# wanmeihuali/taichi_3d_gaussian_splatting

Hardware: NVIDIA H100
Metric: rendered Mpix/sec fwd+bwd @1080p, 1e6 Gaussians (higher is better)
Workload: dtype f32

## Files before the change

taichi_3d_gaussian_splatting_b200/csrc/api.cu:

```cuda
#include <cstdarg>
#include <cstdio>
#include <cstring>

#include "common.cuh"

namespace gsb {

static thread_local char g_error[512] = "";

void set_error(const char *fmt, ...) {
    va_list ap;
    va_start(ap, fmt);
    vsnprintf(g_error, sizeof(g_error), fmt, ap);
    va_end(ap);
}

static inline int64_t align_up(int64_t v, int64_t a) { return (v + a - 1) / a * a; }

static int bit_width(uint64_t v) {
    int b = 0;
    while (v) {
        ++b;
        v >>= 1;
    }
// ... 151 lines not shown
}

using namespace gsb;

extern "C" {

int gsb200_version(void) { return GSB200_VERSION; }

const char *gsb200_last_error(void) { return g_error; }

void gsb200_abi_sizes(int64_t *out3) {
    out3[0] = (int64_t)sizeof(GsbWorkspaceLayout);
    out3[1] = (int64_t)sizeof(GsbForwardArgs);
    out3[2] = (int64_t)sizeof(GsbBackwardArgs);
}

void gsb200_abi_sizes_ext(int64_t *out, int32_t n) {
    const int64_t all[5] = {(int64_t)sizeof(GsbWorkspaceLayout), (int64_t)sizeof(GsbForwardArgs), (int64_t)sizeof(GsbBackwardArgs),
                            (int64_t)sizeof(GsbExpandArgs), (int64_t)sizeof(GsbTrainStepArgs)};
    for (int i = 0; i < n && i < 5; ++i) out[i] = all[i];
}

int gsb200_workspace_layout(int64_t num_points, int32_t num_objects, int64_t key_capacity,
                            int32_t camera_height, int32_t camera_width, float far_plane,
                            float depth_to_sort_key_scale, uint32_t flags, GsbWorkspaceLayout *out) {
    return compute_layout(num_points, num_objects, key_capacity, camera_height, camera_width, far_plane,
                          depth_to_sort_key_scale, flags, out);
}

int gsb200_stage_preprocess(const GsbForwardArgs *a) {
    Workspace ws;
    int rc = resolve_fwd(a, &ws);
    if (rc != GSB_OK) return rc;
    cudaStream_t st = static_cast<cudaStream_t>(a->stream);
    GSB_CUDA_CHECK(cudaMemsetAsync(a->workspace, 0, (size_t)ws.layout.zero_bytes, st));
    return launch_preprocess(*a, ws, st);
}

int gsb200_stage_sort(const GsbForwardArgs *a) {
    Workspace ws;
    int rc = resolve_fwd(a, &ws);
    if (rc != GSB_OK) return rc;
    return launch_sort(ws, a->key_capacity, static_cast<cudaStream_t>(a->stream));
}

int gsb200_stage_tile_ranges(const GsbForwardArgs *a) {
    Workspace ws;
    int rc = resolve_fwd(a, &ws);
    if (rc != GSB_OK) return rc;
    const int T = (a->camera_height / GSB_TILE_HEIGHT) * (a->camera_width / GSB_TILE_WIDTH);
    return launch_tile_ranges(ws, a->key_capacity, T, static_cast<cudaStream_t>(a->stream));
}

int gsb200_stage_blend(const GsbForwardArgs *a) {
    Workspace ws;
    int rc = resolve_fwd(a, &ws);
    if (rc != GSB_OK) return rc;
    return launch_blend_forward(*a, ws, static_cast<cudaStream_t>(a->stream));
}

int gsb200_forward(const GsbForwardArgs *a) {
    Workspace ws;
    int rc = resolve_fwd(a, &ws);
    if (rc != GSB_OK) return rc;
    cudaStream_t st = static_cast<cudaStream_t>(a->stream);
    GSB_CUDA_CHECK(cudaMemsetAsync(a->workspace, 0, (size_t)ws.layout.zero_bytes, st));
    if ((rc = launch_preprocess(*a, ws, st)) != GSB_OK) return rc;
    if (a->host_counters && a->host_counters_event) {
        GSB_CUDA_CHECK(cudaMemcpyAsync(a->host_counters, ws.counters, 4 * sizeof(int64_t), cudaMemcpyDeviceToHost, st));
        GSB_CUDA_CHECK(cudaEventRecord(static_cast<cudaEvent_t>(a->host_counters_event), st));
    }
    if ((rc = launch_sort(ws, a->key_capacity, st)) != GSB_OK) return rc;
    const int T = (a->camera_height / GSB_TILE_HEIGHT) * (a->camera_width / GSB_TILE_WIDTH);
    if ((rc = launch_tile_ranges(ws, a->key_capacity, T, st)) != GSB_OK) return rc;
    return launch_blend_forward(*a, ws, st);
}

static int backward_impl(const GsbBackwardArgs *a, bool skip_on_overflow) {
    if (!a) {
        set_error("backward: args is null");
        return GSB_EINVAL;
    }
    const bool compact = (a->flags & GSB_FLAG_COMPACT_GRADS) != 0;
    if (!a->grad_rasterized_image || !a->pixel_accumulated_alpha ||
        !a->pixel_offset_of_last_effective_point || !a->magnitude_grad_viewspace_on_image ||
        !a->camera_intrinsics ||
        (a->num_points > 0 && (!a->pointcloud || !a->pointcloud_features || !a->point_object_id || !a->t_pointcloud_camera)) ||
        (a->num_points > 0 && !compact && (!a->grad_pointcloud || !a->grad_pointcloud_features)) ||
        (a->num_points > 0 && compact && (!a->grad_sum_compact || !a->grad_color_compact))) {
        set_error("backward: null pointer argument");
        return GSB_EINVAL;
    }
    {
        const void *ctl[6] = {a->ctl_accumulated_num_in_camera, a->ctl_accumulated_num_pixels,
                              a->ctl_accumulated_view_space_position_gradients,
                              a->ctl_accumulated_view_space_position_gradients_avg, a->ctl_accumulated_position_gradients,
                              a->ctl_accumulated_position_gradients_norm};
        int set = 0;
        for (const void *c : ctl) set += c != nullptr;
// ... 87 lines not shown
    cudaStream_t st;
    bool ok = true;
    explicit StageTimer(cudaStream_t s) : st(s) {
        for (auto &e : ev) ok = ok && cudaEventCreate(&e) == cudaSuccess;
    }
    ~StageTimer() {
        for (auto &e : ev) cudaEventDestroy(e);
    }
    void mark() {
        if (n < 9) cudaEventRecord(ev[n++], st);
    }
    int finish(float *out) {
        if (cudaStreamSynchronize(st) != cudaSuccess) return GSB_ECUDA;
        for (int i = 0; i < 8; ++i) out[i] = 0.0f;
        for (int i = 0; i + 1 < n; ++i) cudaEventElapsedTime(&out[i], ev[i], ev[i + 1]);
        return GSB_OK;
    }
};
}

int gsb200_forward_timed(const GsbForwardArgs *a, float *stage_ms_out) {
    Workspace ws;
    int rc = resolve_fwd(a, &ws);
    if (rc != GSB_OK) return rc;
    if (!stage_ms_out) return GSB_EINVAL;
    cudaStream_t st = static_cast<cudaStream_t>(a->stream);
    StageTimer t(st);
    if (!t.ok) {
        set_error("forward_timed: cudaEventCreate failed");
        return GSB_ECUDA;
    }
    const int T = (a->camera_height / GSB_TILE_HEIGHT) * (a->camera_width / GSB_TILE_WIDTH);
    t.mark();
    GSB_CUDA_CHECK(cudaMemsetAsync(a->workspace, 0, (size_t)ws.layout.zero_bytes, st));
    t.mark();
    if ((rc = launch_preprocess(*a, ws, st)) != GSB_OK) return rc;
    t.mark();
    if ((rc = launch_sort(ws, a->key_capacity, st)) != GSB_OK) return rc;
    t.mark();
    if ((rc = launch_tile_ranges(ws, a->key_capacity, T, st)) != GSB_OK) return rc;
    t.mark();
    if ((rc = launch_blend_forward(*a, ws, st)) != GSB_OK) return rc;
    t.mark();
    return t.finish(stage_ms_out);
}

int gsb200_backward_timed(const GsbBackwardArgs *a, float *stage_ms_out) {
    if (!a || !stage_ms_out) return GSB_EINVAL;
    Workspace ws;
    int rc = resolve_workspace(a->workspace, a->workspace_bytes, a->num_points, a->num_objects,
                               a->key_capacity, a->camera_height, a->camera_width, a->far_plane,
                               a->depth_to_sort_key_scale, a->flags, &ws);
    if (rc != GSB_OK) return rc;
    cudaStream_t st = static_cast<cudaStream_t>(a->stream);
    StageTimer t(st);
    if (!t.ok) {
        set_error("backward_timed: cudaEventCreate failed");
        return GSB_ECUDA;
    }
    t.mark();
    if (a->accum_rows > 0)
        GSB_CUDA_CHECK(cudaMemsetAsync(a->accum, 0, (size_t)a->accum_rows * GSB_ACCUM_FLOATS * 4, st));
    t.mark();
    if ((rc = launch_blend_backward(*a, ws, st)) != GSB_OK) return rc;
    t.mark();
    if ((rc = launch_backward_points(*a, ws, st)) != GSB_OK) return rc;
    t.mark();
// ... 99 lines not shown
}

int gsb200_sort_pairs(const void *keys_in, const int32_t *vals_in, void *keys_out, int32_t *vals_out,
                      int64_t n, int32_t key_bytes, int32_t end_bit, void *temp, int64_t temp_bytes,
                      void *stream) {
    if (n < 0 || (key_bytes != 4 && key_bytes != 8) || end_bit < 1 || end_bit > key_bytes * 8) {
        set_error("sort_pairs: bad arguments (n=%lld key_bytes=%d end_bit=%d)", (long long)n, key_bytes, end_bit);
        return GSB_EINVAL;
    }
    if (n == 0) return GSB_OK;
    if (n >= (1LL << 30)) {
        set_error("sort_pairs: n must be < 2^30");
        return GSB_EUNSUPPORTED;
    }
    if (!keys_in || !vals_in || !keys_out || !vals_out || !temp || temp_bytes < gsb200_sort_temp_bytes(n, key_bytes)) {
        set_error("sort_pairs: null pointer or temp too small");
        return GSB_EINVAL;
    }
    if (reinterpret_cast<uintptr_t>(keys_in) % 16 != 0 || reinterpret_cast<uintptr_t>(temp) % 256 != 0) {
        set_error("sort_pairs: keys_in must be 16-byte aligned and temp 256-byte aligned");
        return GSB_EINVAL;
    }
    cudaStream_t st = static_cast<cudaStream_t>(stream);
    const int64_t padded = align_up(n, SORT_TILE);
    const int64_t blocks = padded / SORT_TILE;
    char *b = static_cast<char *>(temp);
    long long *n_dev = reinterpret_cast<long long *>(b);
    unsigned int *tickets = reinterpret_cast<unsigned int *>(b + 256);
    unsigned int *hist = reinterpret_cast<unsigned int *>(b + 512);
    unsigned int *state = reinterpret_cast<unsigned int *>(b + 512 + 8 * 1024 * 4);
    const int64_t state_bytes = align_up(8 * blocks * 1024 * 4, 256);
    void *tmp_keys = b + 512 + 8 * 1024 * 4 + state_bytes;
    int *tmp_vals = reinterpret_cast<int *>(static_cast<char *>(tmp_keys) + align_up(padded * key_bytes, 256));
    GSB_CUDA_CHECK(cudaMemsetAsync(b, 0, (size_t)(512 + 8 * 1024 * 4 + state_bytes), st));
    const long long n_host = n;
    GSB_CUDA_CHECK(cudaMemcpyAsync(n_dev, &n_host, sizeof(n_host), cudaMemcpyHostToDevice, st));
    return sort_pairs_device(keys_in, vals_in, keys_out, vals_out, n_dev, padded, key_bytes, 0, end_bit, nullptr, hist,
                             state, tickets, tmp_keys, tmp_vals, st);
}

int gsb200_render_host(const GsbForwardArgs *device_args, const float *host_q, const float *host_t,
                       const float *host_K, float *staging, float *host_image_out,
                       int64_t *host_counters_out) {
    if (!device_args || !host_q || !host_t || !host_K || !staging || !host_image_out) {
        set_error("render_host: null pointer argument");
        return GSB_EINVAL;
    }
    GsbForwardArgs a = *device_args;
    cudaStream_t st = static_cast<cudaStream_t>(a.stream);
    const int n = a.num_objects;
    float *d_q = staging, *d_t = staging + 4 * n, *d_K = staging + 7 * n;
    GSB_CUDA_CHECK(cudaMemcpyAsync(d_q, host_q, sizeof(float) * 4 * n, cudaMemcpyHostToDevice, st));
    GSB_CUDA_CHECK(cudaMemcpyAsync(d_t, host_t, sizeof(float) * 3 * n, cudaMemcpyHostToDevice, st));
    GSB_CUDA_CHECK(cudaMemcpyAsync(d_K, host_K, sizeof(float) * 9, cudaMemcpyHostToDevice, st));
    a.q_pointcloud_camera = d_q;
    a.t_pointcloud_camera = d_t;
    a.camera_intrinsics = d_K;
    int rc = gsb200_forward(&a);
    if (rc != GSB_OK) return rc;
    GSB_CUDA_CHECK(cudaMemcpyAsync(host_image_out, a.rasterized_image,
                                   sizeof(float) * 3 * (size_t)a.camera_height * a.camera_width,
                                   cudaMemcpyDeviceToHost, st));
    if (host_counters_out)
        GSB_CUDA_CHECK(cudaMemcpyAsync(host_counters_out, a.workspace, sizeof(int64_t) * 4,
                                       cudaMemcpyDeviceToHost, st));
    GSB_CUDA_CHECK(cudaStreamSynchronize(st));
    return GSB_OK;
// ... 4 lines not shown
```

taichi_3d_gaussian_splatting_b200/csrc/common.cuh:

```cuda
#pragma once
#include <cuda_runtime.h>
#include <stdint.h>

#include "../../include/gsb200.h"

#define GSB_TILE_PIXELS (GSB_TILE_WIDTH * GSB_TILE_HEIGHT)

namespace gsb {

void set_error(const char *fmt, ...);
#define GSB_CUDA_CHECK(expr)                                                                   \
    do {                                                                                       \
        cudaError_t _e = (expr);                                                               \
        if (_e != cudaSuccess) {                                                               \
            gsb::set_error("%s failed: %s (%s:%d)", #expr, cudaGetErrorString(_e), __FILE__,   \
                           __LINE__);                                                          \
            return GSB_ECUDA;                                                                  \
        }                                                                                      \
    } while (0)

enum Counter { CNT_M = 0, CNT_K = 1, CNT_OVERFLOW = 2, CNT_MAX_DEPTH_KEY = 4 };
enum Ticket { TICKET_SCAN = 0, TICKET_SORT0 = 1  };

struct PoseBlock {
// ... 146 lines not shown
    return m;
}
#endif

#if defined(__CUDACC__) || defined(GSB_HOST_EMU)
constexpr float GSB_L2E = 1.4426950408889634f;
#ifdef GSB_HOST_EMU
__device__ __forceinline__ float ex2_mufu(float x) { return exp2f(x); }
#else
__device__ __forceinline__ float ex2_mufu(float x) {
    float y;
    asm("ex2.approx.ftz.f32 %0, %1;" : "=f"(y) : "f"(x));
    return y;
}
#endif
__device__ __forceinline__ float fast_alpha(float dx, float dy, float A, float B, float C, float ro) {
    return ex2_mufu(fmaf(dx, fmaf(A, dx, B * dy), (C * dy) * dy)) * ro;
}
__device__ __forceinline__ void fast_planes(const float4 r0, const float4 r1, float4 &s0, float4 &s1) {
    s0 = make_float4(r0.x, r0.y, (-0.5f * GSB_L2E) * r0.z, -GSB_L2E * r0.w);
    s1 = make_float4((-0.5f * GSB_L2E) * r1.x, r1.y * r1.z, 1.0f - r1.z, r1.w);
}
#endif

#if defined(__CUDACC__) || defined(GSB_HOST_EMU)
#ifdef GSB_HOST_EMU
__device__ __forceinline__ void mbar_init(unsigned long long *bar, unsigned int) { *bar = 0; }
__device__ __forceinline__ void mbar_arrive_expect_tx(unsigned long long *, unsigned int) {}
__device__ __forceinline__ void bulk_copy_g2s(void *dst_smem, const void *src_gmem, unsigned int bytes,
                                              unsigned long long *) {
    memcpy(dst_smem, src_gmem, bytes);
}
__device__ __forceinline__ void mbar_wait(unsigned long long *, unsigned int) { simt_emu::warp_exchange(0u); }
#else
__device__ __forceinline__ unsigned int smem_addr(const void *p) {
    return (unsigned int)__cvta_generic_to_shared(p);
}
__device__ __forceinline__ void mbar_init(unsigned long long *bar, unsigned int count) {
    asm volatile("mbarrier.init.shared::cta.b64 [%0], %1;" ::"r"(smem_addr(bar)), "r"(count));
    asm volatile("fence.mbarrier_init.release.cluster;" ::: "memory");
}
__device__ __forceinline__ void mbar_arrive_expect_tx(unsigned long long *bar, unsigned int bytes) {
    asm volatile("mbarrier.arrive.expect_tx.shared::cta.b64 _, [%0], %1;" ::"r"(smem_addr(bar)),
                 "r"(bytes)
                 : "memory");
}
__device__ __forceinline__ void bulk_copy_g2s(void *dst_smem, const void *src_gmem, unsigned int bytes,
                                              unsigned long long *bar) {
    asm volatile(
        "cp.async.bulk.shared::cluster.global.mbarrier::complete_tx::bytes [%0], [%1], %2, [%3];" ::"r"(
            smem_addr(dst_smem)),
        "l"(src_gmem), "r"(bytes), "r"(smem_addr(bar))
        : "memory");
}
__device__ __forceinline__ void mbar_wait(unsigned long long *bar, unsigned int parity) {
    asm volatile(
        "{\n"
        ".reg .pred p;\n"
        "WAIT_LOOP:\n"
        "mbarrier.try_wait.parity.shared::cta.b64 p, [%0], %1;\n"
        "@p bra WAIT_DONE;\n"
        "bra WAIT_LOOP;\n"
        "WAIT_DONE:\n"
        "}\n" ::"r"(smem_addr(bar)),
        "r"(parity)
        : "memory");
}
#endif

#endif

#ifdef GSB_HOST_EMU
#define GSB_EMU_COUNT(slot, n) (simt_emu::counters()[slot] += (long long)(n))
#else
#define GSB_EMU_COUNT(slot, n) ((void)0)
#endif
enum EmuCounter {
    EC_BF_VISITS = 0,
    EC_BF_VISITS_ANY = 1,
    EC_BF_PAIRS = 2,
    EC_TB_SPLATS = 3,
    EC_TB_CHUNKS = 4,
    EC_TB_ROWS = 5,
    EC_BATCHES = 6,
    EC_FW_VISITS = 7,
    EC_FW_PAIRS = 8,
};

static inline int num_sms() {
    static int n = 0;
    if (n == 0) {
        int dev = 0;
        cudaGetDevice(&dev);
        cudaDeviceGetAttribute(&n, cudaDevAttrMultiProcessorCount, dev);
        if (n <= 0) n = 132;
    }
    return n;
}

}
// ... 1 lines not shown
```

taichi_3d_gaussian_splatting_b200/csrc/preprocess.cu:

```cuda
#include "common.cuh"

namespace gsb {

template <int AR, int AC, int BC>
__device__ __forceinline__ void matmul(const float *a, const float *b, float *out) {
#pragma unroll
    for (int i = 0; i < AR; ++i)
#pragma unroll
        for (int j = 0; j < BC; ++j) {
            float s = a[i * AC] * b[j];
#pragma unroll
            for (int k = 1; k < AC; ++k) s = s + a[i * AC + k] * b[k * BC + j];
            out[i * BC + j] = s;
        }
}

__device__ __forceinline__ void rotation_from_quaternion(float x, float y, float z, float w, float *R) {
    float xx = x * x, yy = y * y, zz = z * z;
    float xy = x * y, xz = x * z, yz = y * z;
    float wx = w * x, wy = w * y, wz = w * z;
    R[0] = 1 - 2 * (yy + zz); R[1] = 2 * (xy - wz);     R[2] = 2 * (xz + wy);
    R[3] = 2 * (xy + wz);     R[4] = 1 - 2 * (xx + zz); R[5] = 2 * (yz - wx);
    R[6] = 2 * (xz - wy);     R[7] = 2 * (yz + wx);     R[8] = 1 - 2 * (xx + yy);
}

__device__ __forceinline__ float exp_cr(float x) { return (float)exp((double)x); }
__device__ __forceinline__ float sigmoid_cr(float x) { return 1.0f / (1.0f + exp_cr(-x)); }

__device__ __forceinline__ void quat_mul(const float *a, const float *b, float *o) {
    float x0 = a[0], y0 = a[1], z0 = a[2], w0 = a[3];
    float x1 = b[0], y1 = b[1], z1 = b[2], w1 = b[3];
    o[0] = w0 * x1 + x0 * w1 + y0 * z1 - z0 * y1;
    o[1] = w0 * y1 - x0 * z1 + y0 * w1 + z0 * x1;
    o[2] = w0 * z1 + x0 * y1 - y0 * x1 + z0 * w1;
    o[3] = w0 * w1 - x0 * x1 - y0 * y1 - z0 * z1;
}

__global__ void pose_kernel(const float *__restrict__ q_pc, const float *__restrict__ t_pc, int n_obj,
                            PoseBlock *__restrict__ poses) {
    int o = blockIdx.x * blockDim.x + threadIdx.x;
    if (o >= n_obj) return;
    float qi[4] = {-q_pc[4 * o], -q_pc[4 * o + 1], -q_pc[4 * o + 2], q_pc[4 * o + 3]};
    float t[3] = {t_pc[3 * o], t_pc[3 * o + 1], t_pc[3 * o + 2]};
    float n = sqrtf(((qi[0] * qi[0] + qi[1] * qi[1]) + qi[2] * qi[2]) + qi[3] * qi[3]);
    float qn[4] = {qi[0] / n, qi[1] / n, qi[2] / n, qi[3] / n};
    float v[4] = {t[0], t[1], t[2], 0.0f};
    float qc[4] = {-qn[0], -qn[1], -qn[2], qn[3]};
    float tmp[4], rot[4];
    quat_mul(qn, v, tmp);
    quat_mul(tmp, qc, rot);
    float ti[3] = {-rot[0], -rot[1], -rot[2]};
    float R[9];
    rotation_from_quaternion(qi[0], qi[1], qi[2], qi[3], R);
    PoseBlock pb;
    pb.T[0] = R[0]; pb.T[1] = R[1]; pb.T[2] = R[2];  pb.T[3] = ti[0];
    pb.T[4] = R[3]; pb.T[5] = R[4]; pb.T[6] = R[5];  pb.T[7] = ti[1];
    pb.T[8] = R[6]; pb.T[9] = R[7]; pb.T[10] = R[8]; pb.T[11] = ti[2];
    float nRT[9] = {-R[0], -R[3], -R[6], -R[1], -R[4], -R[7], -R[2], -R[5], -R[8]};
    matmul<3, 3, 1>(nRT, ti, pb.centre);
#pragma unroll
    for (int k = 0; k < 5; ++k) pb.pad[k] = 0.0f;
    poses[o] = pb;
}

constexpr unsigned long long ST_AGGREGATE = 1ull << 62;
constexpr unsigned long long ST_INCLUSIVE = 2ull << 62;
constexpr unsigned long long ST_VALUE_MASK = (1ull << 62) - 1;
constexpr int CNT_SHIFT = 36;

__device__ __forceinline__ unsigned long long ld_state(const unsigned long long *p) {
    return *reinterpret_cast<const volatile unsigned long long *>(p);
}
__device__ __forceinline__ void st_state(unsigned long long *p, unsigned long long v) {
// ... 17 lines not shown
    int W, H;
    float near_plane, far_plane, depth_scale;
    int depth_bits;
    int skip_q_normalise;
    int filter_tiles;
    long long key_capacity;
    long long key_store_limit;
    int num_blocks;
    long long *counters;
    unsigned int *tickets;
    unsigned long long *scan_state;
    int *point_id;
    int *point_offset;
    int *num_tiles;
    float4 *records;
    float *point_in_camera;
    void *keys;
    int *vals;
};

__device__ __forceinline__ void bounding_box(float u, float v, float radii, int W, int H, int &a, int &b,
                                             int &c, int &d) {
    radii = fmaxf(radii, 1.0f);
    float min_u = fmaxf(0.0f, u - radii), max_u = u + radii;
    float min_v = fmaxf(0.0f, v - radii), max_v = v + radii;
    int tw = W / GSB_TILE_WIDTH, th = H / GSB_TILE_HEIGHT;
    a = min((int)floorf(min_u / (float)GSB_TILE_WIDTH), tw);
    b = min(max((int)floorf(max_u / (float)GSB_TILE_WIDTH) + 1, a + 1), tw);
    c = min((int)floorf(min_v / (float)GSB_TILE_HEIGHT), th);
    d = min(max((int)floorf(max_v / (float)GSB_TILE_HEIGHT) + 1, c + 1), th);
}

#ifndef GSB_PRE_MIN_BLOCKS
#define GSB_PRE_MIN_BLOCKS 8
#endif
struct WarpStage {
    float u[32], v[32], a[32], b2[32], c[32], nb_ic[32], nb_ia[32], t2[32];
    int min_tu[32], min_tv[32], ntv[32];
    unsigned int mask_lo[32], mask_hi[32];
    int pref[33];
    int nk64[32], depth_key[32], off[32];
    long long key_base[32];
};

__device__ __forceinline__ int select_bit32(unsigned int m, int j) {
    int pos = 0;
#pragma unroll
    for (int w = 16; w >= 1; w >>= 1) {
        const int c = __popc(m & ((1u << w) - 1u));
        const bool up = j >= c;
        j -= up ? c : 0;
        pos += up ? w : 0;
        m = up ? (m >> w) : m;
    }
    return pos;
}

__device__ __forceinline__ bool tile_reachable(const SplatReach &r, float u, float v, int tu, int tv) {
    const float X0 = (float)(tu * GSB_TILE_WIDTH) + 0.5f - u;
    const float Y0 = (float)(tv * GSB_TILE_HEIGHT) + 0.5f - v;
    return rect_reachable(r, X0, X0 + (float)(GSB_TILE_WIDTH - 1), Y0, Y0 + (float)(GSB_TILE_HEIGHT - 1));
}

template <typename KeyT>
__global__ void __launch_bounds__(SCAN_BLOCK_THREADS, GSB_PRE_MIN_BLOCKS)
preprocess_kernel(const PreParams p) {
    __shared__ unsigned int s_ticket;
// ... 293 lines not shown
        KeyT *keys = reinterpret_cast<KeyT *>(p.keys);
        const int tiles_x = p.W / GSB_TILE_WIDTH;
        for (int q = lane; q < total; q += 32) {
            int lo = 0;
#pragma unroll
            for (int step = 16; step > 0; step >>= 1)
                if (st.pref[lo + step] <= q) lo += step;
            const int j = q - st.pref[lo];
            int idx;
            const int nk64 = st.nk64[lo];
            if (j < nk64) {
                const unsigned int mlo = st.mask_lo[lo];
                const int plo = __popc(mlo);
                idx = j < plo ? select_bit32(mlo, j) : 32 + select_bit32(st.mask_hi[lo], j - plo);
            } else {
                idx = 64 + (j - nk64);
            }
            const int ntv_o = st.ntv[lo];
            const int du = idx / ntv_o;
            const int tu = st.min_tu[lo] + du, tv = st.min_tv[lo] + (idx - du * ntv_o);
            const long long pos = st.key_base[lo] + j;
            if (pos < p.key_store_limit) {
                const KeyT tile = (KeyT)(tu + tv * tiles_x);
                keys[pos] = (tile << p.depth_bits) | (KeyT)(unsigned int)st.depth_key[lo];
                p.vals[pos] = st.off[lo];
            }
        }
    }
}

#ifndef GSB_HOST_EMU
int launch_preprocess(const GsbForwardArgs &a, const Workspace &ws, cudaStream_t stream) {
    const GsbWorkspaceLayout &L = ws.layout;
    if (a.num_objects > 0) {
        const int threads = 64;
        pose_kernel<<<(a.num_objects + threads - 1) / threads, threads, 0, stream>>>(
            a.q_pointcloud_camera, a.t_pointcloud_camera, a.num_objects, ws.poses);
        GSB_CUDA_CHECK(cudaGetLastError());
    }
    if (a.num_points <= 0) return GSB_OK;
    PreParams p;
    p.N = a.num_points;
    p.xyz = a.pointcloud;
    p.features = a.pointcloud_features;
    p.invalid = reinterpret_cast<const signed char *>(a.point_invalid_mask);
    p.obj_id = a.point_object_id;
    p.poses = ws.poses;
    p.K = a.camera_intrinsics;
    p.W = a.camera_width;
    p.H = a.camera_height;
    p.near_plane = a.near_plane;
    p.far_plane = a.far_plane;
    p.depth_scale = a.depth_to_sort_key_scale;
    p.depth_bits = L.depth_bits;
    p.skip_q_normalise = (a.flags & GSB_FLAG_Q_ALREADY_NORMALISED) ? 1 : 0;
    p.filter_tiles = (a.flags & GSB_FLAG_KEEP_ALL_TILE_PAIRS) ? 0 : 1;
    p.key_capacity = a.key_capacity;
    p.key_store_limit = ws.layout.key_capacity_padded;
    p.num_blocks = L.scan_blocks;
    p.counters = ws.counters;
    p.tickets = ws.tickets;
    p.scan_state = ws.scan_state;
    p.point_id = ws.point_id;
    p.point_offset = ws.point_offset;
    p.num_tiles = ws.num_tiles;
    p.records = ws.records;
    p.point_in_camera = ws.point_in_camera;
    p.keys = ws.keys_a;
    p.vals = ws.vals_a;
    if (L.key_bytes == 4)
// ... 10 lines not shown
```

taichi_3d_gaussian_splatting_b200/csrc/sort.cu:

```cuda
#include "common.cuh"

namespace gsb {

constexpr unsigned int SS_AGGREGATE = 1u << 30;
constexpr unsigned int SS_INCLUSIVE = 2u << 30;
constexpr unsigned int SS_VALUE_MASK = (1u << 30) - 1;
#ifndef GSB_SORT_LOOKBACK
#define GSB_SORT_LOOKBACK 4
#endif
constexpr int LOOKBACK = GSB_SORT_LOOKBACK;
constexpr int RBITS = 8;
constexpr int RADIX = 1 << RBITS;
static_assert(RADIX == SORT_BLOCK_THREADS, "one digit per thread");

int sort_radix_bits(int bits) {
    (void)bits;
    return RBITS;
}

__device__ __forceinline__ unsigned int ld_u32_volatile(const unsigned int *p) {
    return *reinterpret_cast<const volatile unsigned int *>(p);
}
__device__ __forceinline__ void st_u32_volatile(unsigned int *p, unsigned int v) {
    *reinterpret_cast<volatile unsigned int *>(p) = v;
}

template <typename KeyT>
struct DigitSel {
    int s_lo, s_hi;
    KeyT m_lo, m_hi;
};
template <typename KeyT>
__device__ __forceinline__ int digit_of(KeyT k, const DigitSel<KeyT> &s) {
    return (int)(((k >> s.s_lo) & s.m_lo) | ((k >> s.s_hi) & s.m_hi));
}
__device__ __forceinline__ int live_depth_bits(const int *max_depth_key, int depth_bits) {
    if (!max_depth_key) return depth_bits;
    unsigned int m = (unsigned int)*max_depth_key;
    int b = 0;
    while (m) {
        ++b;
        m >>= 1;
    }
    return b < depth_bits ? b : depth_bits;
}
__device__ __forceinline__ int active_passes(int end_bit, int depth_bits, int live) {
    const int total = end_bit - depth_bits + live;
    const int p = (total + RBITS - 1) / RBITS;
    return p < 1 ? 1 : p;
}
template <typename KeyT>
__device__ __forceinline__ DigitSel<KeyT> make_digit_sel(int pass, int depth_bits, int live) {
    const int lo = pass * RBITS;
    int n_lo = live - lo;
    n_lo = n_lo < 0 ? 0 : (n_lo > RBITS ? RBITS : n_lo);
    DigitSel<KeyT> s;
    s.s_lo = n_lo > 0 ? lo : 0;
    s.m_lo = (KeyT)((1u << n_lo) - 1u);
    const int first = lo > live ? lo : live;
    const int n_hi = RBITS - n_lo;
    s.s_hi = depth_bits + first - live - n_lo;
    s.m_hi = (KeyT)(((1u << n_hi) - 1u) << n_lo);
    if (s.s_hi > (int)sizeof(KeyT) * 8 - 1) {
        s.s_hi = 0;
        s.m_hi = 0;
    }
    return s;
}

template <typename KeyT>
__global__ void __launch_bounds__(SORT_BLOCK_THREADS)
sort_histogram_kernel(const KeyT *__restrict__ keys, const long long *__restrict__ n_dev, long long capacity,
                      int depth_bits, int end_bit, const int *__restrict__ max_depth_key,
                      unsigned int *__restrict__ hist, unsigned int *__restrict__ done_ctr) {
    __shared__ unsigned int s_hist[8 * RADIX];
    __shared__ unsigned int s_scan[SORT_BLOCK_THREADS / 32];
    __shared__ unsigned int s_last;
    const int tid = threadIdx.x, lane = tid & 31, warp = tid >> 5;
    const int live = live_depth_bits(max_depth_key, depth_bits);
    const int passes = active_passes(end_bit, depth_bits, live);
    for (int i = tid; i < passes * RADIX; i += SORT_BLOCK_THREADS) s_hist[i] = 0;
    __syncthreads();
    long long n = *n_dev;
    if (n > capacity) n = capacity;
    DigitSel<KeyT> sel[8];
#pragma unroll
    for (int p = 0; p < 8; ++p) sel[p] = make_digit_sel<KeyT>(p, depth_bits, live);
    constexpr int VEC = 16 / (int)sizeof(KeyT), HIST_U = 2;
    const long long stride = (long long)gridDim.x * SORT_BLOCK_THREADS;
    const long long nvec = n / VEC;
    const uint4 *const kv = reinterpret_cast<const uint4 *>(keys);
    for (long long i = (long long)blockIdx.x * SORT_BLOCK_THREADS + tid; i < nvec; i += HIST_U * stride) {
        uint4 v[HIST_U];
#pragma unroll
        for (int u = 0; u < HIST_U; ++u)
            if (i + u * stride < nvec) v[u] = kv[i + u * stride];
#pragma unroll
        for (int u = 0; u < HIST_U; ++u) {
            if (i + u * stride >= nvec) continue;
            KeyT kk[VEC];
            if (sizeof(KeyT) == 4) {
                kk[0] = (KeyT)v[u].x; kk[1] = (KeyT)v[u].y; kk[VEC - 2] = (KeyT)v[u].z; kk[VEC - 1] = (KeyT)v[u].w;
            } else {
                kk[0] = (KeyT)v[u].x | ((KeyT)v[u].y << (4 * sizeof(KeyT)));
                kk[VEC - 1] = (KeyT)v[u].z | ((KeyT)v[u].w << (4 * sizeof(KeyT)));
            }
#pragma unroll
            for (int e = 0; e < VEC; ++e)
#pragma unroll
                for (int p = 0; p < 8; ++p)
                    if (p < passes) atomicAdd(&s_hist[p * RADIX + digit_of(kk[e], sel[p])], 1u);
        }
    }
    for (long long i = nvec * VEC + (long long)blockIdx.x * SORT_BLOCK_THREADS + tid; i < n; i += stride) {
        const KeyT k = keys[i];
#pragma unroll
        for (int p = 0; p < 8; ++p)
// ... 48 lines not shown
    KeyT *keys_b;
    int *vals_b;
    KeyT *keys_c;
    int *vals_c;
    const long long *n_dev;
    long long capacity;
    int pass, depth_bits, end_bit, blocks;
    const int *max_depth_key;
    const unsigned int *hist;
    unsigned int *state;
    unsigned int *tickets;
};

#ifndef GSB_HOST_EMU
extern __shared__ __align__(128) unsigned char gsb_sort_dynamic_smem[];
#endif

template <typename KeyT>
__global__ void __launch_bounds__(SORT_BLOCK_THREADS, GSB_SORT_MIN_BLOCKS)
onesweep_pass_kernel(const PassParams<KeyT> P) {
#ifdef GSB_HOST_EMU
    PassSmem<KeyT> &s = *reinterpret_cast<PassSmem<KeyT> *>(
        (reinterpret_cast<uintptr_t>(simt_emu::dynamic_smem()) + 127) & ~uintptr_t(127));
#else
    PassSmem<KeyT> &s = *reinterpret_cast<PassSmem<KeyT> *>(gsb_sort_dynamic_smem);
#endif
    const int tid = threadIdx.x, lane = tid & 31, warp = tid >> 5;

    const int live = live_depth_bits(P.max_depth_key, P.depth_bits);
    const int npass = active_passes(P.end_bit, P.depth_bits, live);
    if (P.pass >= npass) return;
    long long n = *P.n_dev;
    if (n > P.capacity) n = P.capacity;
    if (tid == 0) s.ticket = atomicAdd(P.tickets + P.pass, 1u);
    __syncthreads();
    const unsigned int blk = s.ticket;
    const long long tile_base = (long long)blk * SORT_TILE;
    if (tile_base >= n) return;
    const int count = (int)min((long long)SORT_TILE, n - tile_base);
    const DigitSel<KeyT> sel = make_digit_sel<KeyT>(P.pass, P.depth_bits, live);
    const bool to_b = ((npass - 1 - P.pass) & 1) == 0;
    const KeyT *const keys_in = P.pass == 0 ? P.keys_a : (to_b ? P.keys_c : P.keys_b);
    const int *const vals_in = P.pass == 0 ? P.vals_a : (to_b ? P.vals_c : P.vals_b);
    KeyT *const keys_out = to_b ? P.keys_b : P.keys_c;
    int *const vals_out = to_b ? P.vals_b : P.vals_c;
    const unsigned int *const hist = P.hist + P.pass * RADIX;
    unsigned int *const state = P.state + (size_t)P.pass * P.blocks * RADIX;

    if (tid == 0) mbar_init(&s.mbar, 1);
    {
        unsigned int *z = reinterpret_cast<unsigned int *>(&s.warp_cnt[0][0]);
#pragma unroll
        for (int i = 0; i < (SORT_BLOCK_THREADS / 32) * RADIX / 2 / SORT_BLOCK_THREADS; ++i) z[i * SORT_BLOCK_THREADS + tid] = 0;
    }
    __syncthreads();

    const unsigned int bulk_bytes = ((unsigned int)count * (unsigned int)sizeof(KeyT)) & ~15u;
    const int bulk_elems = (int)(bulk_bytes / sizeof(KeyT));
    if (tid == 0 && bulk_bytes) {
        mbar_arrive_expect_tx(&s.mbar, bulk_bytes);
        bulk_copy_g2s(s.keys, keys_in + tile_base, bulk_bytes, &s.mbar);
    }
    if (bulk_elems + tid < count) s.keys[bulk_elems + tid] = keys_in[tile_base + bulk_elems + tid];
    int vals[SORT_ITEMS_PER_THREAD];
    const int wbase = warp * (32 * SORT_ITEMS_PER_THREAD);
    {
        const int *vp = vals_in + tile_base + wbase + lane;
#pragma unroll
        for (int j = 0; j < SORT_ITEMS_PER_THREAD; ++j)
            vals[j] = wbase + j * 32 + lane < count ? __ldg(vp + j * 32) : 0;
    }
    if (bulk_bytes) mbar_wait(&s.mbar, 0);
    __syncthreads();

    KeyT keys[SORT_ITEMS_PER_THREAD];
    unsigned short ranks[SORT_ITEMS_PER_THREAD];
    const unsigned int lt_mask = (1u << lane) - 1u;
    unsigned short *const my_cnt = s.warp_cnt[warp];
#pragma unroll
    for (int j = 0; j < SORT_ITEMS_PER_THREAD; ++j) {
        const int idx = wbase + j * 32 + lane;
        const bool valid = idx < count;
        keys[j] = s.keys[idx];
        const int d = valid ? digit_of(keys[j], sel) : RADIX;
        const unsigned int peers = __match_any_sync(0xffffffffu, d);
        unsigned int prev = 0;
        if (valid) prev = my_cnt[d];
        ranks[j] = (unsigned short)(prev + __popc(peers & lt_mask));
        __syncwarp();
        if (valid && (peers & lt_mask) == 0) my_cnt[d] = (unsigned short)(prev + __popc(peers));
        __syncwarp();
    }
    __syncthreads();

    unsigned int cnt = 0;
#pragma unroll
    for (int w = 0; w < SORT_BLOCK_THREADS / 32; ++w) {
        const unsigned int x = s.warp_cnt[w][tid];
        s.warp_cnt[w][tid] = (unsigned short)cnt;
        cnt += x;
    }
    unsigned int *const my_state = state + (size_t)blk * RADIX + tid;
    st_u32_volatile(my_state, (blk == 0 ? SS_INCLUSIVE : SS_AGGREGATE) | cnt);
    {
        unsigned int incl = cnt;
#pragma unroll
        for (int d = 1; d < 32; d <<= 1) {
            const unsigned int o = __shfl_up_sync(0xffffffffu, incl, d);
            if (lane >= d) incl += o;
        }
        if (lane == 31) s.scan_tmp[warp] = incl;
        __syncthreads();
        unsigned int wprefix = 0;
#pragma unroll
        for (int w = 0; w < SORT_BLOCK_THREADS / 32; ++w)
            if (w < warp) wprefix += s.scan_tmp[w];
        s.digit_start[tid] = wprefix + incl - cnt;
    }
    const unsigned int dglobal = hist[tid];
    __syncthreads();

#pragma unroll
    for (int j = 0; j < SORT_ITEMS_PER_THREAD; ++j) {
        const int idx = wbase + j * 32 + lane;
        if (idx < count) {
            const int d = digit_of(keys[j], sel);
            const unsigned int pos = s.digit_start[d] + my_cnt[d] + ranks[j];
            s.keys[pos] = keys[j];
            s.vals[pos] = vals[j];
        }
    }

    unsigned int excl = 0;
    if (blk != 0) {
        int look = (int)blk - 1;
        const unsigned int *const col = state + tid;
        bool done = false;
        while (!done) {
            unsigned int w[LOOKBACK];
#pragma unroll
            for (int r = 0; r < LOOKBACK; ++r)
                w[r] = (look - r >= 0) ? ld_u32_volatile(col + (size_t)(look - r) * RADIX) : SS_INCLUSIVE;
#pragma unroll
            for (int r = 0; r < LOOKBACK; ++r) {
                if (done) continue;
                while ((w[r] >> 30) == 0) w[r] = ld_u32_volatile(col + (size_t)(look - r) * RADIX);
                excl += w[r] & SS_VALUE_MASK;
                done = (w[r] >> 30) == 2;
            }
            look -= LOOKBACK;
        }
        st_u32_volatile(my_state, SS_INCLUSIVE | (excl + cnt));
    }
    s.global_base[tid] = dglobal + excl - s.digit_start[tid];
    __syncthreads();

#pragma unroll
    for (int j = 0; j < SORT_ITEMS_PER_THREAD; ++j) {
        const int pidx = j * SORT_BLOCK_THREADS + tid;
        if (pidx < count) {
            const KeyT k = s.keys[pidx];
            const unsigned int dst = s.global_base[digit_of(k, sel)] + (unsigned int)pidx;
            keys_out[dst] = k;
            vals_out[dst] = s.vals[pidx];
        }
    }
}

#ifndef GSB_HOST_EMU
template <typename KeyT>
static int sort_pairs_typed(const KeyT *keys_in, const int *vals_in, KeyT *keys_out, int *vals_out,
                            const long long *n_dev, int64_t capacity, int depth_bits, int end_bit,
                            const int *max_depth_key, unsigned int *hist, unsigned int *state, unsigned int *tickets,
                            KeyT *tmp_keys, int *tmp_vals, cudaStream_t stream) {
    const int passes = (end_bit + RBITS - 1) / RBITS;
    const int blocks = (int)((capacity + SORT_TILE - 1) / SORT_TILE);
    if (blocks == 0 || passes == 0) return GSB_OK;
    const size_t smem = sizeof(PassSmem<KeyT>);
    static bool attr_set = false;
    if (!attr_set) {
        GSB_CUDA_CHECK(cudaFuncSetAttribute(onesweep_pass_kernel<KeyT>, cudaFuncAttributeMaxDynamicSharedMemorySize,
                                            (int)smem));
        attr_set = true;
    }
#ifndef GSB_HIST_BLOCKS_PER_SM
#define GSB_HIST_BLOCKS_PER_SM 4
#endif
    int hist_blocks = blocks < GSB_HIST_BLOCKS_PER_SM * num_sms() ? blocks : GSB_HIST_BLOCKS_PER_SM * num_sms();
    sort_histogram_kernel<KeyT><<<hist_blocks, SORT_BLOCK_THREADS, 0, stream>>>(keys_in, n_dev, capacity, depth_bits, end_bit,
                                                                                  max_depth_key, hist, tickets + 8);
    GSB_CUDA_CHECK(cudaGetLastError());
    PassParams<KeyT> P;
    P.keys_a = keys_in;
    P.vals_a = vals_in;
    P.keys_b = keys_out;
    P.vals_b = vals_out;
    P.keys_c = tmp_keys;
    P.vals_c = tmp_vals;
    P.n_dev = n_dev;
    P.capacity = capacity;
    P.depth_bits = depth_bits;
    P.end_bit = end_bit;
    P.blocks = blocks;
    P.max_depth_key = max_depth_key;
    P.hist = hist;
    P.state = state;
    P.tickets = tickets;
    for (int p = 0; p < passes; ++p) {
        P.pass = p;
        onesweep_pass_kernel<KeyT><<<blocks, SORT_BLOCK_THREADS, smem, stream>>>(P);
        GSB_CUDA_CHECK(cudaGetLastError());
    }
    return GSB_OK;
}

int sort_pairs_device(const void *keys_in, const int *vals_in, void *keys_out, int *vals_out,
                      const long long *n_dev, int64_t n_capacity, int key_bytes, int depth_bits, int end_bit,
                      const int *max_depth_key, unsigned int *hist, unsigned int *state, unsigned int *tickets,
                      void *tmp_keys, int *tmp_vals, cudaStream_t stream) {
    typedef unsigned int u32;
    typedef unsigned long long u64;
    if (depth_bits < 0 || depth_bits > end_bit) {
        set_error("sort: depth_bits %d outside [0, end_bit = %d]", depth_bits, end_bit);
        return GSB_EINVAL;
    }
    if (key_bytes == 4)
        return sort_pairs_typed<u32>((const u32 *)keys_in, vals_in, (u32 *)keys_out, vals_out, n_dev, n_capacity, depth_bits,
                                     end_bit, max_depth_key, hist, state, tickets, (u32 *)tmp_keys, tmp_vals, stream);
    if (key_bytes == 8)
        return sort_pairs_typed<u64>((const u64 *)keys_in, vals_in, (u64 *)keys_out, vals_out, n_dev, n_capacity, depth_bits,
                                     end_bit, max_depth_key, hist, state, tickets, (u64 *)tmp_keys, tmp_vals, stream);
    set_error("sort: key_bytes must be 4 or 8, got %d", key_bytes);
    return GSB_EINVAL;
}

#endif

template <typename KeyT>
__global__ void __launch_bounds__(256)
tile_ranges_kernel(const KeyT *__restrict__ keys, const long long *__restrict__ n_dev, long long capacity,
                   int depth_bits, int num_tiles, int *__restrict__ tile_start,
                   int *__restrict__ tile_end) {
    long long n = n_dev ? *n_dev : capacity;
// ... 60 lines not shown
```

Measured before the change: 1199.

## Fold workspace clearing into kernels and make onesweep sort persistent

```diff
diff --git a/taichi_3d_gaussian_splatting_b200/csrc/api.cu b/taichi_3d_gaussian_splatting_b200/csrc/api.cu
--- a/taichi_3d_gaussian_splatting_b200/csrc/api.cu
+++ b/taichi_3d_gaussian_splatting_b200/csrc/api.cu
@@ -207,9 +207,7 @@
     Workspace ws;
     int rc = resolve_fwd(a, &ws);
     if (rc != GSB_OK) return rc;
-    cudaStream_t st = static_cast<cudaStream_t>(a->stream);
-    GSB_CUDA_CHECK(cudaMemsetAsync(a->workspace, 0, (size_t)ws.layout.zero_bytes, st));
-    return launch_preprocess(*a, ws, st);
+    return launch_preprocess(*a, ws, static_cast<cudaStream_t>(a->stream));
 }
 
 int gsb200_stage_sort(const GsbForwardArgs *a) {
@@ -239,7 +237,6 @@
     int rc = resolve_fwd(a, &ws);
     if (rc != GSB_OK) return rc;
     cudaStream_t st = static_cast<cudaStream_t>(a->stream);
-    GSB_CUDA_CHECK(cudaMemsetAsync(a->workspace, 0, (size_t)ws.layout.zero_bytes, st));
     if ((rc = launch_preprocess(*a, ws, st)) != GSB_OK) return rc;
     if (a->host_counters && a->host_counters_event) {
         GSB_CUDA_CHECK(cudaMemcpyAsync(a->host_counters, ws.counters, 4 * sizeof(int64_t), cudaMemcpyDeviceToHost, st));
@@ -393,7 +390,6 @@
     }
     const int T = (a->camera_height / GSB_TILE_HEIGHT) * (a->camera_width / GSB_TILE_WIDTH);
     t.mark();
-    GSB_CUDA_CHECK(cudaMemsetAsync(a->workspace, 0, (size_t)ws.layout.zero_bytes, st));
     t.mark();
     if ((rc = launch_preprocess(*a, ws, st)) != GSB_OK) return rc;
     t.mark();
@@ -559,7 +555,7 @@
     const int64_t state_bytes = align_up(8 * blocks * 1024 * 4, 256);
     void *tmp_keys = b + 512 + 8 * 1024 * 4 + state_bytes;
     int *tmp_vals = reinterpret_cast<int *>(static_cast<char *>(tmp_keys) + align_up(padded * key_bytes, 256));
-    GSB_CUDA_CHECK(cudaMemsetAsync(b, 0, (size_t)(512 + 8 * 1024 * 4 + state_bytes), st));
+    GSB_CUDA_CHECK(cudaMemsetAsync(b, 0, (size_t)(512 + 8 * 1024 * 4), st));
     const long long n_host = n;
     GSB_CUDA_CHECK(cudaMemcpyAsync(n_dev, &n_host, sizeof(n_host), cudaMemcpyHostToDevice, st));
     return sort_pairs_device(keys_in, vals_in, keys_out, vals_out, n_dev, padded, key_bytes, 0, end_bit, nullptr, hist,
diff --git a/taichi_3d_gaussian_splatting_b200/csrc/common.cuh b/taichi_3d_gaussian_splatting_b200/csrc/common.cuh
--- a/taichi_3d_gaussian_splatting_b200/csrc/common.cuh
+++ b/taichi_3d_gaussian_splatting_b200/csrc/common.cuh
@@ -202,6 +202,7 @@
     memcpy(dst_smem, src_gmem, bytes);
 }
 __device__ __forceinline__ void mbar_wait(unsigned long long *, unsigned int) { simt_emu::warp_exchange(0u); }
+__device__ __forceinline__ void fence_proxy_async_smem() {}
 #else
 __device__ __forceinline__ unsigned int smem_addr(const void *p) {
     return (unsigned int)__cvta_generic_to_shared(p);
@@ -236,6 +237,7 @@
         "r"(parity)
         : "memory");
 }
+__device__ __forceinline__ void fence_proxy_async_smem() { asm volatile("fence.proxy.async.shared::cta;" ::: "memory"); }
 #endif
 
 #endif
diff --git a/taichi_3d_gaussian_splatting_b200/csrc/preprocess.cu b/taichi_3d_gaussian_splatting_b200/csrc/preprocess.cu
--- a/taichi_3d_gaussian_splatting_b200/csrc/preprocess.cu
+++ b/taichi_3d_gaussian_splatting_b200/csrc/preprocess.cu
@@ -37,8 +37,12 @@
 }
 
 __global__ void pose_kernel(const float *__restrict__ q_pc, const float *__restrict__ t_pc, int n_obj,
-                            PoseBlock *__restrict__ poses) {
-    int o = blockIdx.x * blockDim.x + threadIdx.x;
+                            PoseBlock *__restrict__ poses, uint4 *__restrict__ clear0 = nullptr, int clear0_vec = 0,
+                            uint4 *__restrict__ clear1 = nullptr, int clear1_vec = 0) {
+    const int o = blockIdx.x * blockDim.x + threadIdx.x;
+    const int stride = gridDim.x * blockDim.x;
+    for (int k = o; k < clear0_vec; k += stride) clear0[k] = make_uint4(0u, 0u, 0u, 0u);
+    for (int k = o; k < clear1_vec; k += stride) clear1[k] = make_uint4(0u, 0u, 0u, 0u);
     if (o >= n_obj) return;
     float qi[4] = {-q_pc[4 * o], -q_pc[4 * o + 1], -q_pc[4 * o + 2], q_pc[4 * o + 3]};
     float t[3] = {t_pc[3 * o], t_pc[3 * o + 1], t_pc[3 * o + 2]};
@@ -122,7 +126,7 @@
 }
 
 #ifndef GSB_PRE_MIN_BLOCKS
-#define GSB_PRE_MIN_BLOCKS 8
+#define GSB_PRE_MIN_BLOCKS 5
 #endif
 struct WarpStage {
     float u[32], v[32], a[32], b2[32], c[32], nb_ic[32], nb_ia[32], t2[32];
@@ -482,10 +486,16 @@
 #ifndef GSB_HOST_EMU
 int launch_preprocess(const GsbForwardArgs &a, const Workspace &ws, cudaStream_t stream) {
     const GsbWorkspaceLayout &L = ws.layout;
-    if (a.num_objects > 0) {
+    {
+        const int clear0_vec = (int)((L.sort_state - L.counters) / 16), clear1_vec = (int)((L.zero_bytes - L.tile_start) / 16);
         const int threads = 64;
-        pose_kernel<<<(a.num_objects + threads - 1) / threads, threads, 0, stream>>>(
-            a.q_pointcloud_camera, a.t_pointcloud_camera, a.num_objects, ws.poses);
+        const int pose_blocks = (a.num_objects + threads - 1) / threads;
+        int clear_blocks = (clear0_vec + clear1_vec + 4 * threads - 1) / (4 * threads);
+        if (clear_blocks > 4 * num_sms()) clear_blocks = 4 * num_sms();
+        const int blocks = pose_blocks > clear_blocks ? pose_blocks : clear_blocks;
+        pose_kernel<<<blocks > 0 ? blocks : 1, threads, 0, stream>>>(
+            a.q_pointcloud_camera, a.t_pointcloud_camera, a.num_objects, ws.poses,
+            reinterpret_cast<uint4 *>(ws.counters), clear0_vec, reinterpret_cast<uint4 *>(ws.tile_start), clear1_vec);
         GSB_CUDA_CHECK(cudaGetLastError());
     }
     if (a.num_points <= 0) return GSB_OK;
diff --git a/taichi_3d_gaussian_splatting_b200/csrc/sort.cu b/taichi_3d_gaussian_splatting_b200/csrc/sort.cu
--- a/taichi_3d_gaussian_splatting_b200/csrc/sort.cu
+++ b/taichi_3d_gaussian_splatting_b200/csrc/sort.cu
@@ -23,6 +23,17 @@
 }
 __device__ __forceinline__ void st_u32_volatile(unsigned int *p, unsigned int v) {
     *reinterpret_cast<volatile unsigned int *>(p) = v;
+}
+
+__device__ __forceinline__ unsigned int match_digit(int v) {
+    unsigned int peers = 0xffffffffu;
+#pragma unroll
+    for (int b = 0; b <= RBITS; ++b) {
+        const bool bit = (v >> b) & 1;
+        const unsigned int set = __ballot_sync(0xffffffffu, bit);
+        peers &= bit ? set : ~set;
+    }
+    return peers;
 }
 
 template <typename KeyT>
@@ -72,7 +83,8 @@
 __global__ void __launch_bounds__(SORT_BLOCK_THREADS)
 sort_histogram_kernel(const KeyT *__restrict__ keys, const long long *__restrict__ n_dev, long long capacity,
                       int depth_bits, int end_bit, const int *__restrict__ max_depth_key,
-                      unsigned int *__restrict__ hist, unsigned int *__restrict__ done_ctr) {
+                      unsigned int *__restrict__ hist, unsigned int *__restrict__ done_ctr,
+                      unsigned int *__restrict__ state = nullptr, long long state_pass_words = 0) {
     __shared__ unsigned int s_hist[8 * RADIX];
     __shared__ unsigned int s_scan[SORT_BLOCK_THREADS / 32];
     __shared__ unsigned int s_last;
@@ -83,6 +95,14 @@
     __syncthreads();
     long long n = *n_dev;
     if (n > capacity) n = capacity;
+    if (state) {
+        const long long per_pass = (n + SORT_TILE - 1) / SORT_TILE * (RADIX / 4);
+        for (long long k = (long long)blockIdx.x * SORT_BLOCK_THREADS + tid; k < passes * per_pass;
+             k += (long long)gridDim.x * SORT_BLOCK_THREADS) {
+            const long long p = k / per_pass;
+            reinterpret_cast<uint4 *>(state + p * state_pass_words)[k - p * per_pass] = make_uint4(0u, 0u, 0u, 0u);
+        }
+    }
     DigitSel<KeyT> sel[8];
 #pragma unroll
     for (int p = 0; p < 8; ++p) sel[p] = make_digit_sel<KeyT>(p, depth_bits, live);
@@ -197,12 +217,6 @@
     if (P.pass >= npass) return;
     long long n = *P.n_dev;
     if (n > P.capacity) n = P.capacity;
-    if (tid == 0) s.ticket = atomicAdd(P.tickets + P.pass, 1u);
-    __syncthreads();
-    const unsigned int blk = s.ticket;
-    const long long tile_base = (long long)blk * SORT_TILE;
-    if (tile_base >= n) return;
-    const int count = (int)min((long long)SORT_TILE, n - tile_base);
     const DigitSel<KeyT> sel = make_digit_sel<KeyT>(P.pass, P.depth_bits, live);
     const bool to_b = ((npass - 1 - P.pass) & 1) == 0;
     const KeyT *const keys_in = P.pass == 0 ? P.keys_a : (to_b ? P.keys_c : P.keys_b);
@@ -211,124 +225,137 @@
     int *const vals_out = to_b ? P.vals_b : P.vals_c;
     const unsigned int *const hist = P.hist + P.pass * RADIX;
     unsigned int *const state = P.state + (size_t)P.pass * P.blocks * RADIX;
-
     if (tid == 0) mbar_init(&s.mbar, 1);
-    {
-        unsigned int *z = reinterpret_cast<unsigned int *>(&s.warp_cnt[0][0]);
-#pragma unroll
-        for (int i = 0; i < (SORT_BLOCK_THREADS / 32) * RADIX / 2 / SORT_BLOCK_THREADS; ++i) z[i * SORT_BLOCK_THREADS + tid] = 0;
-    }
-    __syncthreads();
-
-    const unsigned int bulk_bytes = ((unsigned int)count * (unsigned int)sizeof(KeyT)) & ~15u;
-    const int bulk_elems = (int)(bulk_bytes / sizeof(KeyT));
-    if (tid == 0 && bulk_bytes) {
-        mbar_arrive_expect_tx(&s.mbar, bulk_bytes);
-        bulk_copy_g2s(s.keys, keys_in + tile_base, bulk_bytes, &s.mbar);
-    }
-    if (bulk_elems + tid < count) s.keys[bulk_elems + tid] = keys_in[tile_base + bulk_elems + tid];
-    int vals[SORT_ITEMS_PER_THREAD];
-    const int wbase = warp * (32 * SORT_ITEMS_PER_THREAD);
-    {
-        const int *vp = vals_in + tile_base + wbase + lane;
-#pragma unroll
-        for (int j = 0; j < SORT_ITEMS_PER_THREAD; ++j)
-            vals[j] = wbase + j * 32 + lane < count ? __ldg(vp + j * 32) : 0;
-    }
-    if (bulk_bytes) mbar_wait(&s.mbar, 0);
-    __syncthreads();
-
-    KeyT keys[SORT_ITEMS_PER_THREAD];
-    unsigned short ranks[SORT_ITEMS_PER_THREAD];
-    const unsigned int lt_mask = (1u << lane) - 1u;
-    unsigned short *const my_cnt = s.warp_cnt[warp];
-#pragma unroll
-    for (int j = 0; j < SORT_ITEMS_PER_THREAD; ++j) {
-        const int idx = wbase + j * 32 + lane;
-        const bool valid = idx < count;
-        keys[j] = s.keys[idx];
-        const int d = valid ? digit_of(keys[j], sel) : RADIX;
-        const unsigned int peers = __match_any_sync(0xffffffffu, d);
-        unsigned int prev = 0;
-        if (valid) prev = my_cnt[d];
-        ranks[j] = (unsigned short)(prev + __popc(peers & lt_mask));
-        __syncwarp();
-        if (valid && (peers & lt_mask) == 0) my_cnt[d] = (unsigned short)(prev + __popc(peers));
-        __syncwarp();
-    }
-    __syncthreads();
-
-    unsigned int cnt = 0;
-#pragma unroll
-    for (int w = 0; w < SORT_BLOCK_THREADS / 32; ++w) {
-        const unsigned int x = s.warp_cnt[w][tid];
-        s.warp_cnt[w][tid] = (unsigned short)cnt;
-        cnt += x;
-    }
-    unsigned int *const my_state = state + (size_t)blk * RADIX + tid;
-    st_u32_volatile(my_state, (blk == 0 ? SS_INCLUSIVE : SS_AGGREGATE) | cnt);
-    {
-        unsigned int incl = cnt;
-#pragma unroll
-        for (int d = 1; d < 32; d <<= 1) {
-            const unsigned int o = __shfl_up_sync(0xffffffffu, incl, d);
-            if (lane >= d) incl += o;
-        }
-        if (lane == 31) s.scan_tmp[warp] = incl;
-        __syncthreads();
-        unsigned int wprefix = 0;
-#pragma unroll
-        for (int w = 0; w < SORT_BLOCK_THREADS / 32; ++w)
-            if (w < warp) wprefix += s.scan_tmp[w];
-        s.digit_start[tid] = wprefix + incl - cnt;
-    }
-    const unsigned int dglobal = hist[tid];
-    __syncthreads();
-
-#pragma unroll
-    for (int j = 0; j < SORT_ITEMS_PER_THREAD; ++j) {
-        const int idx = wbase + j * 32 + lane;
-        if (idx < count) {
-            const int d = digit_of(keys[j], sel);
-            const unsigned int pos = s.digit_start[d] + my_cnt[d] + ranks[j];
-            s.keys[pos] = keys[j];
-            s.vals[pos] = vals[j];
-        }
-    }
-
-    unsigned int excl = 0;
-    if (blk != 0) {
-        int look = (int)blk - 1;
-        const unsigned int *const col = state + tid;
-        bool done = false;
-        while (!done) {
-            unsigned int w[LOOKBACK];
-#pragma unroll
-            for (int r = 0; r < LOOKBACK; ++r)
-                w[r] = (look - r >= 0) ? ld_u32_volatile(col + (size_t)(look - r) * RADIX) : SS_INCLUSIVE;
-#pragma unroll
-            for (int r = 0; r < LOOKBACK; ++r) {
-                if (done) continue;
-                while ((w[r] >> 30) == 0) w[r] = ld_u32_volatile(col + (size_t)(look - r) * RADIX);
-                excl += w[r] & SS_VALUE_MASK;
-                done = (w[r] >> 30) == 2;
+    unsigned int phase = 0;
+
+    for (;;) {
+        if (tid == 0) s.ticket = atomicAdd(P.tickets + P.pass, 1u);
+        {
+            unsigned int *z = reinterpret_cast<unsigned int *>(&s.warp_cnt[0][0]);
+#pragma unroll
+            for (int i = 0; i < (SORT_BLOCK_THREADS / 32) * RADIX / 2 / SORT_BLOCK_THREADS; ++i) z[i * SORT_BLOCK_THREADS + tid] = 0;
+        }
+        __syncthreads();
+        const unsigned int blk = s.ticket;
+        const long long tile_base = (long long)blk * SORT_TILE;
+        if (tile_base >= n) return;
+        const int count = (int)min((long long)SORT_TILE, n - tile_base);
+
+        const unsigned int bulk_bytes = ((unsigned int)count * (unsigned int)sizeof(KeyT)) & ~15u;
+        const int bulk_elems = (int)(bulk_bytes / sizeof(KeyT));
+        if (tid == 0 && bulk_bytes) {
+            fence_proxy_async_smem();
+            mbar_arrive_expect_tx(&s.mbar, bulk_bytes);
+            bulk_copy_g2s(s.keys, keys_in + tile_base, bulk_bytes, &s.mbar);
+        }
+        if (bulk_elems + tid < count) s.keys[bulk_elems + tid] = keys_in[tile_base + bulk_elems + tid];
+        int vals[SORT_ITEMS_PER_THREAD];
+        const int wbase = warp * (32 * SORT_ITEMS_PER_THREAD);
+        {
+            const int *vp = vals_in + tile_base + wbase + lane;
+#pragma unroll
+            for (int j = 0; j < SORT_ITEMS_PER_THREAD; ++j)
+                vals[j] = wbase + j * 32 + lane < count ? __ldg(vp + j * 32) : 0;
+        }
+        if (bulk_bytes) {
+            mbar_wait(&s.mbar, phase);
+            phase ^= 1u;
+        }
+        __syncthreads();
+
+        KeyT keys[SORT_ITEMS_PER_THREAD];
+        unsigned short ranks[SORT_ITEMS_PER_THREAD];
+        const unsigned int lt_mask = (1u << lane) - 1u;
+        unsigned short *const my_cnt = s.warp_cnt[warp];
+#pragma unroll
+        for (int j = 0; j < SORT_ITEMS_PER_THREAD; ++j) {
+            const int idx = wbase + j * 32 + lane;
+            const bool valid = idx < count;
+            keys[j] = s.keys[idx];
+            const int d = valid ? digit_of(keys[j], sel) : RADIX;
+            const unsigned int peers = match_digit(d);
+            unsigned int prev = 0;
+            if (valid) prev = my_cnt[d];
+            ranks[j] = (unsigned short)(prev + __popc(peers & lt_mask));
+            __syncwarp();
+            if (valid && (peers & lt_mask) == 0) my_cnt[d] = (unsigned short)(prev + __popc(peers));
+            __syncwarp();
+        }
+        __syncthreads();
+
+        unsigned int cnt = 0;
+#pragma unroll
+        for (int w = 0; w < SORT_BLOCK_THREADS / 32; ++w) {
+            const unsigned int x = s.warp_cnt[w][tid];
+            s.warp_cnt[w][tid] = (unsigned short)cnt;
+            cnt += x;
+        }
+        unsigned int *const my_state = state + (size_t)blk * RADIX + tid;
+        st_u32_volatile(my_state, (blk == 0 ? SS_INCLUSIVE : SS_AGGREGATE) | cnt);
+        {
+            unsigned int incl = cnt;
+#pragma unroll
+            for (int d = 1; d < 32; d <<= 1) {
+                const unsigned int o = __shfl_up_sync(0xffffffffu, incl, d);
+                if (lane >= d) incl += o;
             }
-            look -= LOOKBACK;
-        }
-        st_u32_volatile(my_state, SS_INCLUSIVE | (excl + cnt));
-    }
-    s.global_base[tid] = dglobal + excl - s.digit_start[tid];
-    __syncthreads();
-
-#pragma unroll
-    for (int j = 0; j < SORT_ITEMS_PER_THREAD; ++j) {
-        const int pidx = j * SORT_BLOCK_THREADS + tid;
-        if (pidx < count) {
-            const KeyT k = s.keys[pidx];
-            const unsigned int dst = s.global_base[digit_of(k, sel)] + (unsigned int)pidx;
-            keys_out[dst] = k;
-            vals_out[dst] = s.vals[pidx];
-        }
+            if (lane == 31) s.scan_tmp[warp] = incl;
+            __syncthreads();
+            unsigned int wprefix = 0;
+#pragma unroll
+            for (int w = 0; w < SORT_BLOCK_THREADS / 32; ++w)
+                if (w < warp) wprefix += s.scan_tmp[w];
+            s.digit_start[tid] = wprefix + incl - cnt;
+        }
+        const unsigned int dglobal = hist[tid];
+        __syncthreads();
+
+#pragma unroll
+        for (int j = 0; j < SORT_ITEMS_PER_THREAD; ++j) {
+            const int idx = wbase + j * 32 + lane;
+            if (idx < count) {
+                const int d = digit_of(keys[j], sel);
+                const unsigned int pos = s.digit_start[d] + my_cnt[d] + ranks[j];
+                s.keys[pos] = keys[j];
+                s.vals[pos] = vals[j];
+            }
+        }
+
+        unsigned int excl = 0;
+        if (blk != 0) {
+            int look = (int)blk - 1;
+            const unsigned int *const col = state + tid;
+            bool done = false;
+            while (!done) {
+                unsigned int w[LOOKBACK];
+#pragma unroll
+                for (int r = 0; r < LOOKBACK; ++r)
+                    w[r] = (look - r >= 0) ? ld_u32_volatile(col + (size_t)(look - r) * RADIX) : SS_INCLUSIVE;
+#pragma unroll
+                for (int r = 0; r < LOOKBACK; ++r) {
+                    if (done) continue;
+                    while ((w[r] >> 30) == 0) w[r] = ld_u32_volatile(col + (size_t)(look - r) * RADIX);
+                    excl += w[r] & SS_VALUE_MASK;
+                    done = (w[r] >> 30) == 2;
+                }
+                look -= LOOKBACK;
+            }
+            st_u32_volatile(my_state, SS_INCLUSIVE | (excl + cnt));
+        }
+        s.global_base[tid] = dglobal + excl - s.digit_start[tid];
+        __syncthreads();
+
+#pragma unroll
+        for (int j = 0; j < SORT_ITEMS_PER_THREAD; ++j) {
+            const int pidx = j * SORT_BLOCK_THREADS + tid;
+            if (pidx < count) {
+                const KeyT k = s.keys[pidx];
+                const unsigned int dst = s.global_base[digit_of(k, sel)] + (unsigned int)pidx;
+                keys_out[dst] = k;
+                vals_out[dst] = s.vals[pidx];
+            }
+        }
+        __syncthreads();
     }
 }
 
@@ -342,18 +369,23 @@
     const int blocks = (int)((capacity + SORT_TILE - 1) / SORT_TILE);
     if (blocks == 0 || passes == 0) return GSB_OK;
     const size_t smem = sizeof(PassSmem<KeyT>);
-    static bool attr_set = false;
-    if (!attr_set) {
+    static int resident = 0;
+    if (!resident) {
         GSB_CUDA_CHECK(cudaFuncSetAttribute(onesweep_pass_kernel<KeyT>, cudaFuncAttributeMaxDynamicSharedMemorySize,
                                             (int)smem));
-        attr_set = true;
-    }
+        int per_sm = 0;
+        GSB_CUDA_CHECK(cudaOccupancyMaxActiveBlocksPerMultiprocessor(&per_sm, onesweep_pass_kernel<KeyT>,
+                                                                     SORT_BLOCK_THREADS, smem));
+        resident = (per_sm > 0 ? per_sm : 1) * num_sms();
+    }
+    const int pass_blocks = blocks < resident ? blocks : resident;
 #ifndef GSB_HIST_BLOCKS_PER_SM
 #define GSB_HIST_BLOCKS_PER_SM 4
 #endif
     int hist_blocks = blocks < GSB_HIST_BLOCKS_PER_SM * num_sms() ? blocks : GSB_HIST_BLOCKS_PER_SM * num_sms();
     sort_histogram_kernel<KeyT><<<hist_blocks, SORT_BLOCK_THREADS, 0, stream>>>(keys_in, n_dev, capacity, depth_bits, end_bit,
-                                                                                  max_depth_key, hist, tickets + 8);
+                                                                                  max_depth_key, hist, tickets + 8, state,
+                                                                                  (long long)blocks * RADIX);
     GSB_CUDA_CHECK(cudaGetLastError());
     PassParams<KeyT> P;
     P.keys_a = keys_in;
@@ -373,7 +405,7 @@
     P.tickets = tickets;
     for (int p = 0; p < passes; ++p) {
         P.pass = p;
-        onesweep_pass_kernel<KeyT><<<blocks, SORT_BLOCK_THREADS, smem, stream>>>(P);
+        onesweep_pass_kernel<KeyT><<<pass_blocks, SORT_BLOCK_THREADS, smem, stream>>>(P);
         GSB_CUDA_CHECK(cudaGetLastError());
     }
     return GSB_OK;
```

After: 1244, median of 6. +3.8%, better.
